# CristianSimion5/vk-raytracing-engine

Hardware: AMD Instinct MI355X
Metric: Mrays/s (higher is better)
Workload: dtype f32

## Files before the change

vk-raytracing-engine_amd/csrc/multihit.hip:

```cpp
#include <hip/hip_runtime.h>

#include "device_math.h"
#include "device_scene.h"
#include "kernels.h"
#include "query_common.h"
#include "traverse.h"
#include "traverse_wide.h"
#include "wf_streams.h"
#include "wide_node.h"

struct MultiList
{
  int* p;
  int K, cnt;
  float boundT;
  int boundGid;

  VKRT_DEV int& word(int f, int j) const { return p[(f * K + j) * 64]; }
  VKRT_DEV void begin(int* lanePtr, int k, float tmax)
  {
    p = lanePtr; K = k; cnt = 0; boundT = tmax; boundGid = -1;
  }
  VKRT_DEV bool admits(float t, int gid) const { return t < boundT || (t == boundT && gid < boundGid); }
  VKRT_DEV void insert(float t, int gid, int slot, float u, float v)
// ... 74 lines not shown
  tr.set(d);
  const float4* __restrict__ nodes = sc.nodes;
  const float4* __restrict__ tris = sc.tris;
  const int cap = (int)(sc.stackCap >> 1);
  const f3 id = mk3(safe_inv(d.x), safe_inv(d.y), safe_inv(d.z));
  const bool px = !(id.x < 0.0f), py = !(id.y < 0.0f), pz = !(id.z < 0.0f);
  const unsigned octinv = (px ? 1u : 0u) | (py ? 2u : 0u) | (pz ? 4u : 0u);
  uint2 G = make_uint2(0u, sc.rootRef == VKRT_TRAV_DONE ? 0u : 0x80000000u);
  int sp = 0;
  unsigned steps = sc.stepLimit;
  TravCount tc;
  while(G.y & 0xff000000u)
  {
    const unsigned bitIdx = 31u - (unsigned)__clz((int)G.y);
    const unsigned slot = (bitIdx - 24u) ^ octinv;
    const unsigned child = G.x + (unsigned)__popc(G.y & 0xffu & ((1u << slot) - 1u));
    G.y &= ~(1u << bitIdx);
    if(G.y & 0xff000000u)
    {
      if(sp < cap)
      {
        stk[sp * stride] = G;
        sp++;
      }
      else
        VKRT_TRAV_FAULT(sc);
    }
    if(--steps == 0u)
    {
      VKRT_TRAV_FAULT(sc);
      return;
    }
    uint2 T;
    w8_test_children<false, (TM & VKRT_TM_FILTER) != 0>(nodes, child, o, id, octinv * 0x01010101u, px, py, pz, tmin, L.boundT, G, T, tc,
                                                        query_node_masks<TM>(sc), query_cull_mask<TM>(sc));
    while(T.y != 0u)
    {
      const unsigned i = (unsigned)__ffs((int)T.y) - 1u;
      T.y &= T.y - 1u;
      if(--steps == 0u)
      {
        VKRT_TRAV_FAULT(sc);
        return;
      }
      multi_test_triangle<TM>(sc, tr, o, d, tmin, T.x + i, tris, L, raySeed);
    }
    if((G.y & 0xff000000u) == 0u)
    {
      if(sp == 0)
        return;
      sp--;
      G = stk[sp * stride];
    }
  }
}

template <bool WIDE, int TM>
__global__ __launch_bounds__(64)
void k_query_multi(const DevQueryScene sc, const float4* __restrict__ rays, uint64_t first, uint64_t n, uint32_t seed, int maxHits,
                   float4* __restrict__ hits, int* __restrict__ counts)
{
  extern __shared__ int lds_multi[];
  const uint64_t i = first + (uint64_t)blockIdx.x * 64u + threadIdx.x;
  if(i >= n)
    return;
  const float4 r0 = wfLoad(rays + 2 * i), r1 = wfLoad(rays + 2 * i + 1);
  const bool valid = queryRayValid(r0, r1) && (!(TM & VKRT_TM_FILTER) || sc.cullMask != 0u);
// ... 39 lines not shown
```

vk-raytracing-engine_amd/csrc/query.hip:

```cpp
#include <hip/hip_runtime.h>
#include <string.h>

#include "device_math.h"
#include "device_scene.h"
#include "kernels.h"
#include "query_common.h"
#include "traverse.h"
#include "traverse_wide.h"
#include "traverse_share.h"
#include "wf_streams.h"
#include "wide_node.h"

template <bool ANYHIT, bool WIDE, int TM>
__global__ __launch_bounds__(64)
__attribute__((amdgpu_waves_per_eu(TM != 0 && WIDE ? 5 : 1)))
void k_query(const DevQueryScene sc, const float4* __restrict__ rays, uint64_t first, uint64_t n, uint32_t seed, float4* __restrict__ hits,
             int* __restrict__ occ)
{
  extern __shared__ int lds_stack[];
  __shared__ int shareLds[VKRT_SHARE_LDS_WORDS];
  const uint64_t i = first + (uint64_t)blockIdx.x * 64u + threadIdx.x;
  const bool inRange = i < n;
  float4 r0 = make_float4(0.0f, 0.0f, 0.0f, 0.0f), r1 = make_float4(1.0f, 0.0f, 0.0f, 0.0f);
  if(inRange)
  {
    r0 = wfLoad(rays + 2 * i);
    r1 = wfLoad(rays + 2 * i + 1);
  }
  const bool valid = inRange && queryRayValid(r0, r1) && (!(TM & VKRT_TM_FILTER) || sc.cullMask != 0u);
  const unsigned long long validMask = __ballot(valid);
  RayHit hit;
  hit.t = r1.w; hit.u = 0.0f; hit.v = 0.0f; hit.slot = -1;
  TravCount tc;
  if(validMask != 0ull)
  {
    const f3 o = valid ? mk3(r0.x, r0.y, r0.z) : mk3(0.0f, 0.0f, 0.0f);
    const f3 d = valid ? mk3(r1.x, r1.y, r1.z) : mk3(1.0f, 0.0f, 0.0f);
    const float tmax = valid ? r1.w : 0.0f;
    const float tmin0 = __shfl(r0.w, __ffsll((long long)validMask) - 1);
    const bool share = WIDE && sc.shareMinIdle != 0u && sc.triThreshold != 0u && __ballot(valid && r0.w != tmin0) == 0ull;
    if(share)
    {
      uint2* stk = ((uint2*)lds_stack) + threadIdx.x;
      traverse_wide8_share<false, ANYHIT, TM>(sc, valid, o, d, tmin0, tmax, stk, shareRes(shareLds), hit, tc, seed);
    }
    else if(valid)
      traverse_any<false, WIDE, TM>(sc, o, d, r0.w, tmax, ANYHIT, lds_stack, (int)threadIdx.x, 64, hit, tc, seed);
  }
// ... 113 lines not shown
```

vk-raytracing-engine_amd/csrc/traverse_share.h:

```cpp
#pragma once
#include "traverse_wide.h"

#define VKRT_SHARE_LDS_WORDS 384
struct ShareRes
{
  unsigned long long* key;
  int* slot;
  float* u;
  float* v;
  int* donor;
};
VKRT_DEV void shareSync()
{
  __builtin_amdgcn_fence(__ATOMIC_RELEASE, "wavefront");
  __builtin_amdgcn_wave_barrier();
  __builtin_amdgcn_fence(__ATOMIC_ACQUIRE, "wavefront");
}
VKRT_DEV unsigned laneRank(unsigned long long mask)
{
  return __builtin_amdgcn_mbcnt_hi((unsigned)(mask >> 32), __builtin_amdgcn_mbcnt_lo((unsigned)mask, 0u));
}
VKRT_DEV ShareRes shareRes(int* lds320)
{
  ShareRes r;
  r.key = (unsigned long long*)lds320; r.slot = lds320 + 128; r.u = (float*)(lds320 + 192); r.v = (float*)(lds320 + 256); r.donor = lds320 + 320;
  return r;
}

template <bool COUNT, bool ANYHIT, int TM = 0>
VKRT_DEV void traverse_wide8_share(const DevScene& sc, bool valid, f3 o, f3 d, float tmin, float tmax, uint2* stk, ShareRes res, RayHit& hit,
                                   TravCount& tc, uint32_t raySeed = 0u)
{
  TriRay<(TM & VKRT_TM_WATERTIGHT) != 0> tr;
  tr.set(d);
  const float4* __restrict__ nodes = sc.nodes;
  const float4* __restrict__ tris = sc.tris;
  const int stride = 64;
  const int cap = (int)(sc.stackCap >> 1);
  const int lane = (int)lane_id();
  const unsigned shareMin = sc.shareMinIdle;
  bool farFirst = ANYHIT && anyhit_far_first(sc, o, d, tmax);

  res.key[lane] = ((unsigned long long)__float_as_uint(tmax) << 32) | 0xffffffffull;
  res.slot[lane] = -1; res.u[lane] = 0.0f; res.v[lane] = 0.0f;
  shareSync();

  int owner = lane;
  f3 id = mk3(safe_inv(d.x), safe_inv(d.y), safe_inv(d.z));
  bool px = !(id.x < 0.0f), py = !(id.y < 0.0f), pz = !(id.z < 0.0f);
  unsigned oct4 = ((px ? 1u : 0u) | (py ? 2u : 0u) | (pz ? 4u : 0u)) * 0x01010101u;
  uint2 G = make_uint2(0u, (valid && sc.rootRef != VKRT_TRAV_DONE) ? 0x80000000u : 0u);
  uint2 T = make_uint2(0u, 0u);
  int sp = 0, sb = 0, nPost = 0;
  unsigned steps = sc.stepLimit;
  bool busy = G.y != 0u;
  const bool lendOn = (TM & (VKRT_TM_WATERTIGHT | VKRT_TM_DISSOLVE)) != (VKRT_TM_WATERTIGHT | VKRT_TM_DISSOLVE) && (sc.shareFlags & VKRT_SHARE_TRI_LEND) != 0u;

  for(unsigned iter = 0;; iter++)
  {
    const unsigned long long busyMask = __ballot(busy);
    if(busyMask == 0ull)
      break;
    if((iter & sc.sharePeriodMask) == sc.sharePeriodMask && (unsigned)__popcll(~busyMask) >= shareMin)
    {
      const bool giveStack = busy && sp - sb >= 1;
      const bool giveChild = (sc.shareFlags & 1u) != 0u && busy && !giveStack && (G.y & 0xff000000u & ((G.y & 0xff000000u) - 1u)) != 0u;
      const bool mayTris = (sc.shareFlags & 16u) != 0u && busy && !giveStack && !giveChild;
      const bool giveParked = mayTris && nPost > 0;
      const bool giveTris = mayTris && !giveParked && (T.y & (T.y - 1u)) != 0u;
      const bool wants = giveStack || giveChild || giveParked || giveTris;
      const unsigned long long donorMask = __ballot(wants), idleMask = ~busyMask;
      if(donorMask != 0ull)
      {
        const unsigned n = min((unsigned)__popcll(donorMask), (unsigned)__popcll(idleMask));
        const unsigned giveRank = laneRank(donorMask), takeRank = laneRank(idleMask);
        const bool gives = wants && giveRank < n;
        const bool takes = !busy && takeRank < n;
        uint2 e = make_uint2(0u, 0u);
        if(gives)
        {
          if(giveStack)
          {
            e = stk[sb * stride];
            sb++;
          }
          else if(giveChild)
          {
            const unsigned top = G.y & 0xff000000u;
            const unsigned low = farFirst ? (0x80000000u >> (unsigned)__clz((int)top)) : (top & (0u - top));
            e = make_uint2(G.x, low | (G.y & 0xffu));
            G.y &= ~low;
          }
          else if(giveParked)
          {
            e = stk[(cap - nPost) * stride];
            e.x |= 0x80000000u;
            nPost--;
          }
          else
          {
            const unsigned lo = (unsigned)__ffs((int)T.y) - 1u, hi = 31u - (unsigned)__clz((int)T.y);
            const unsigned upper = T.y & ~((1u << ((lo + hi + 1u) >> 1)) - 1u);
            e = make_uint2(T.x | 0x80000000u, upper);
            T.y &= ~upper;
          }
          res.donor[giveRank] = lane;
        }
        shareSync();
        const int src = takes ? res.donor[takeRank] : lane;
        const unsigned ex = (unsigned)__shfl((int)e.x, src), ey = (unsigned)__shfl((int)e.y, src);
        const float ox = __shfl(o.x, src), oy = __shfl(o.y, src), oz = __shfl(o.z, src);
        const float dx = __shfl(d.x, src), dy = __shfl(d.y, src), dz = __shfl(d.z, src);
        const float ix = __shfl(id.x, src), iy = __shfl(id.y, src), iz = __shfl(id.z, src);
        const float tm = __shfl(tmax, src);
        const int ow = __shfl(owner, src);
        if(TM & VKRT_TM_DISSOLVE)
        {
          const uint32_t sd = (uint32_t)__shfl((int)raySeed, src);
          if(takes) raySeed = sd;
        }
        if(takes)
        {
          o = mk3(ox, oy, oz); d = mk3(dx, dy, dz); id = mk3(ix, iy, iz); tmax = tm;
          tr.set(d);
          farFirst = ANYHIT && anyhit_far_first(sc, o, d, tmax);
          px = !(id.x < 0.0f); py = !(id.y < 0.0f); pz = !(id.z < 0.0f);
          oct4 = ((px ? 1u : 0u) | (py ? 2u : 0u) | (pz ? 4u : 0u)) * 0x01010101u;
          if(ex & 0x80000000u)
          {
            G = make_uint2(0u, 0u);
            T = make_uint2(ex & 0x7fffffffu, ey);
          }
          else
          {
            G = make_uint2(ex, ey);
            T = make_uint2(0u, 0u);
          }
          sp = 0; sb = 0; nPost = 0;
          owner = ow;
          steps = sc.stepLimit;
          busy = true;
        }
      }
    }
    shareSync();
    if(busy || lendOn)
    {
      float bt = tmax;
      int bg = -1;
      bool finished = false;
      bool occluded = false;
      if(ANYHIT)
        finished = busy && __hip_atomic_load(&res.slot[owner], __ATOMIC_RELAXED, __HIP_MEMORY_SCOPE_WAVEFRONT) >= 0;
      else
      {
        const unsigned long long k = __hip_atomic_load(&res.key[owner], __ATOMIC_RELAXED, __HIP_MEMORY_SCOPE_WAVEFRONT);
        bt = __uint_as_float((unsigned)(k >> 32));
        bg = (int)(unsigned)k;
      }
      if(!finished)
      {
        struct Cand
        {
          bool found;
          float t, u, v;
          int slot, gid;
        };
        auto testOne = [&](Cand& cd) {
          const unsigned i = (unsigned)__ffs((int)T.y) - 1u;
          T.y &= T.y - 1u;
          const unsigned s = T.x + i;
          const float4* __restrict__ tp = tris + (size_t)s * VKRT_TRI_QUADS;
          const float4 a = tp[0];
          const float4 b = tp[1];
          const float4 c = tp[2];
          if(COUNT)
          {
            tc.tris++;
            if(lane == __ffsll((long long)__ballot(1)) - 1) tc.waveTriSteps++;
          }
          float t, u, v;
          bool ccw;
          if(tr.hit(o, d, a, b, c, t, u, v, ccw) && t > tmin)
          {
            if(ANYHIT)
            {
              if(t < tmax && !cd.found && !query_rejects<TM>(sc, c, ccw) && !anyhit_ignores<TM>(sc, s, c.y, raySeed, VKRT_HOOK_UV(TM, u, v)))
              {
                cd.found = true; cd.t = t; cd.slot = (int)s;
              }
            }
            else
            {
              const int gid = tri_gid<TM>(c.y);
              const float rt = cd.found ? cd.t : bt;
              const int rg = cd.found ? cd.gid : bg;
              if((t < rt || (t == rt && gid < rg)) && !query_rejects<TM>(sc, c, ccw) && !anyhit_ignores<TM>(sc, s, c.y, raySeed, VKRT_HOOK_UV(TM, u, v)))
              {
                cd.found = true; cd.t = t; cd.u = u; cd.v = v; cd.slot = (int)s; cd.gid = gid;
              }
            }
          }
        };
        auto publish = [&](const Cand& cd) {
          if(!cd.found)
            return;
          if(ANYHIT)
          {
            __hip_atomic_store(&res.slot[owner], cd.slot, __ATOMIC_RELAXED, __HIP_MEMORY_SCOPE_WAVEFRONT);
            occluded = true;
          }
          else
          {
            const unsigned long long mine = ((unsigned long long)__float_as_uint(cd.t) << 32) | (unsigned)cd.gid;
            __hip_atomic_fetch_min(&res.key[owner], mine, __ATOMIC_RELAXED, __HIP_MEMORY_SCOPE_WAVEFRONT);
            shareSync();
            if(__hip_atomic_load(&res.key[owner], __ATOMIC_RELAXED, __HIP_MEMORY_SCOPE_WAVEFRONT) == mine)
            {
              res.slot[owner] = cd.slot; res.u[owner] = cd.u; res.v[owner] = cd.v;
            }
            bt = cd.t; bg = cd.gid;
          }
        };
        auto flushT = [&]() {
          Cand cd = {false, 0.0f, 0.0f, 0.0f, -1, 0};
          while(T.y != 0u && !(ANYHIT && cd.found))
            testOne(cd);
          publish(cd);
        };
        if(G.y & 0xff000000u)
        {
          const unsigned bitIdx = farFirst ? (unsigned)__ffs((int)(G.y & 0xff000000u)) - 1u : 31u - (unsigned)__clz((int)G.y);
          const unsigned slot = (bitIdx - 24u) ^ (oct4 & 7u);
          const unsigned child = G.x + (unsigned)__popc(G.y & 0xffu & ((1u << slot) - 1u));
          G.y &= ~(1u << bitIdx);
          if(G.y & 0xff000000u)
          {
            if(__builtin_expect(sp + nPost >= cap && nPost > VKRT_W8_POSTPONE_ROOM, 0))
            {
              const uint2 keep = T;
              T = stk[(cap - nPost) * stride];
              nPost--;
              flushT();
              T = keep;
            }
            if(sp + nPost < cap)
            {
              stk[sp * stride] = G;
              sp++;
            }
            else
              VKRT_TRAV_FAULT(sc);
          }
          uint2 Tn;
          w8_test_children<COUNT, (TM & VKRT_TM_FILTER) != 0>(nodes, child, o, id, oct4, px, py, pz, tmin, bt, G, Tn, tc, query_node_masks<TM>(sc),
                                                              query_cull_mask<TM>(sc));
          if(Tn.y != 0u)
          {
            if(T.y != 0u)
            {
              if(__builtin_expect(nPost < VKRT_W8_MAX_POSTPONED && sp + nPost < cap, 1))
              {
                nPost++;
                stk[(cap - nPost) * stride] = T;
              }
              else
              {
                if(!occluded)
                  flushT();
                T.y = 0u;
              }
            }
            T = Tn;
          }
        }
        if((G.y & 0xff000000u) == 0u && sp > sb)
        {
          sp--;
          G = stk[sp * stride];
        }
        if(T.y == 0u && nPost > 0)
        {
          T = stk[(cap - nPost) * stride];
          nPost--;
        }
        bool triStep = true;
        if(sc.triThreshold > 1u)
          triStep = (unsigned)__popcll(__ballot(T.y != 0u)) * 64u >= sc.triThreshold * (unsigned)__popcll(busyMask) ||
                    __ballot((G.y & 0xff000000u) != 0u) == 0ull;
        bool lentStep = false;
        if(lendOn && triStep)
        {
          const bool tests = T.y != 0u && !occluded;
          const unsigned rest1 = T.y & (T.y - 1u);
          const bool multi = rest1 != 0u && !occluded, isFree = T.y == 0u && !occluded;
          const unsigned long long lendMask = __ballot(multi), freeMask = __ballot(isFree);
          const unsigned n = min((unsigned)__popcll(lendMask), (unsigned)__popcll(freeMask));
          if(n != 0u)
          {
            lentStep = true;
            const unsigned lendRank = laneRank(lendMask), freeRank = laneRank(freeMask);
            const bool borrows = isFree && freeRank < n;
            unsigned s = 0u, ls = 0u;
            if(multi && lendRank < n)
            {
              const unsigned hi = 31u - (unsigned)__clz((int)T.y);
              T.y &= ~(1u << hi);
              ls = T.x + hi;
              res.donor[lendRank] = lane;
            }
            if(tests)
            {
              s = T.x + (unsigned)__ffs((int)T.y) - 1u;
              T.y &= T.y - 1u;
            }
            shareSync();
            const int src = borrows ? res.donor[freeRank] : lane;
            const unsigned bs = (unsigned)__shfl((int)ls, src);
            const f3 ro = mk3(__shfl(o.x, src), __shfl(o.y, src), __shfl(o.z, src));
            const f3 rd = mk3(__shfl(d.x, src), __shfl(d.y, src), __shfl(d.z, src));
            const int row = __shfl(owner, src);
            const float rbt = __shfl(bt, src);
            const int rbg = ANYHIT ? 0 : __shfl(bg, src);
            uint32_t rseed = raySeed;
            if(TM & VKRT_TM_DISSOLVE)
              rseed = (uint32_t)__shfl((int)raySeed, src);
            if(tests || borrows)
            {
              if(borrows)
              {
                s = bs;
                tr.set(rd);
              }
              const float4* __restrict__ tp = tris + (size_t)s * VKRT_TRI_QUADS;
              const float4 a = tp[0];
              const float4 b = tp[1];
              const float4 c = tp[2];
              if(COUNT)
              {
                tc.tris++;
                if(lane == __ffsll((long long)__ballot(1)) - 1) tc.waveTriSteps++;
              }
              float t, u, v;
              bool ccw;
              if(tr.hit(ro, rd, a, b, c, t, u, v, ccw) && t > tmin)
              {
                if(ANYHIT)
                {
                  if(t < rbt && !query_rejects<TM>(sc, c, ccw) && !anyhit_ignores<TM>(sc, s, c.y, rseed, VKRT_HOOK_UV(TM, u, v)))
                  {
                    __hip_atomic_store(&res.slot[row], (int)s, __ATOMIC_RELAXED, __HIP_MEMORY_SCOPE_WAVEFRONT);
                    if(!borrows)
                      occluded = true;
                  }
                }
                else
                {
                  const int gid = tri_gid<TM>(c.y);
                  if((t < rbt || (t == rbt && gid < rbg)) && !query_rejects<TM>(sc, c, ccw) && !anyhit_ignores<TM>(sc, s, c.y, rseed, VKRT_HOOK_UV(TM, u, v)))
                  {
                    const unsigned long long mine = ((unsigned long long)__float_as_uint(t) << 32) | (unsigned)gid;
                    __hip_atomic_fetch_min(&res.key[row], mine, __ATOMIC_RELAXED, __HIP_MEMORY_SCOPE_WAVEFRONT);
                    shareSync();
                    if(__hip_atomic_load(&res.key[row], __ATOMIC_RELAXED, __HIP_MEMORY_SCOPE_WAVEFRONT) == mine)
                    {
                      res.slot[row] = (int)s; res.u[row] = u; res.v[row] = v;
                    }
                  }
                }
              }
              if((TM & VKRT_TM_WATERTIGHT) != 0 && borrows)
                tr.set(d);
            }
          }
        }
        if(!lentStep && T.y != 0u && triStep && !occluded)
        {
          Cand cd = {false, 0.0f, 0.0f, 0.0f, -1, 0};
          testOne(cd);
          publish(cd);
        }
        if(ANYHIT && occluded)
          finished = true;
        else if((G.y & 0xff000000u) == 0u && T.y == 0u && nPost == 0)
          finished = true;
        else if(--steps == 0u)
        {
          VKRT_TRAV_FAULT(sc);
          finished = true;
        }
      }
      if(finished)
      {
        if(lendOn && busy)
        {
          G.y = 0u; T.y = 0u; sp = 0; sb = 0; nPost = 0;
        }
        busy = false;
      }
    }
  }
  shareSync();
  hit.t = __uint_as_float((unsigned)(res.key[lane] >> 32)); hit.u = res.u[lane]; hit.v = res.v[lane]; hit.slot = res.slot[lane];
  if(ANYHIT)
    hit.t = tmax;
}
```

vk-raytracing-engine_amd/csrc/traverse_wide.h:

```cpp
#pragma once
#include "device_math.h"
#include "device_scene.h"
#include "traverse.h"
#include "wide_node.h"

typedef float vkrt_v4f __attribute__((ext_vector_type(4)));
VKRT_DEV float ubyte_f32(unsigned w, int k) { return (float)((w >> (8 * k)) & 0xffu); }

template <int TM>
struct W8State
{
  TriRay<(TM & VKRT_TM_WATERTIGHT) != 0> tr;
  uint32_t raySeed;
  bool farFirst;
  f3 o, d, id;
  float tmax, bestT, bestU, bestV;
  int bestSlot, bestGid;
  uint2 G;
  int sp;
  unsigned steps;
  bool anyHit;
};

template <int TM>
VKRT_DEV void w8_begin(const DevScene& sc, W8State<TM>& S, f3 o, f3 d, float tmax, bool anyHit, uint32_t raySeed)
{
  S.o = o; S.d = d;
  S.tr.set(d);
  S.raySeed = raySeed;
  S.farFirst = anyHit && anyhit_far_first(sc, o, d, tmax);
  S.id = mk3(safe_inv(d.x), safe_inv(d.y), safe_inv(d.z));
  S.tmax = tmax; S.bestT = tmax; S.bestU = 0.0f; S.bestV = 0.0f;
  S.bestSlot = -1; S.bestGid = -1;
  S.G = make_uint2(0u, sc.rootRef == VKRT_TRAV_DONE ? 0u : 0x80000000u);
  S.sp = 0;
  S.steps = sc.stepLimit;
  S.anyHit = anyHit;
}

VKRT_DEV unsigned w8_piece(unsigned idx4, unsigned bits4, int k)
{
#if defined(__HIP_DEVICE_COMPILE__) && !defined(__GFX9__)
  return ((bits4 >> (8 * k)) & 0xffu) << ((idx4 >> (8 * k)) & 31u);
#else
  unsigned r;
  if(k == 0)
    asm("v_lshlrev_b32_sdwa %0, %1, %2 dst_sel:DWORD dst_unused:UNUSED_PAD src0_sel:BYTE_0 src1_sel:BYTE_0" : "=v"(r) : "v"(idx4), "v"(bits4));
  else if(k == 1)
    asm("v_lshlrev_b32_sdwa %0, %1, %2 dst_sel:DWORD dst_unused:UNUSED_PAD src0_sel:BYTE_1 src1_sel:BYTE_1" : "=v"(r) : "v"(idx4), "v"(bits4));
  else if(k == 2)
    asm("v_lshlrev_b32_sdwa %0, %1, %2 dst_sel:DWORD dst_unused:UNUSED_PAD src0_sel:BYTE_2 src1_sel:BYTE_2" : "=v"(r) : "v"(idx4), "v"(bits4));
  else
    asm("v_lshlrev_b32_sdwa %0, %1, %2 dst_sel:DWORD dst_unused:UNUSED_PAD src0_sel:BYTE_3 src1_sel:BYTE_3" : "=v"(r) : "v"(idx4), "v"(bits4));
  return r;
#endif
}

template <bool COUNT, bool CULL = false>
VKRT_DEV void w8_test_children(const float4* __restrict__ nodes, unsigned child, f3 o, f3 id, unsigned oct4, bool px, bool py, bool pz, float tmin,
                               float bestT_in, uint2& G, uint2& T, TravCount& tc, const uint2* __restrict__ nodeMasks = nullptr,
                               unsigned cullMask = 0xffu)
{
  const float4* __restrict__ np = nodes + (size_t)child * VKRT_WNODE_QUADS;
  const float4 q0 = np[0], q1 = np[1], q2 = np[2], q3 = np[3], q4 = np[4];
  uint2 slotMasks = make_uint2(0xffffffffu, 0xffffffffu);
  if(CULL)
    slotMasks = nodeMasks[child];
  if(COUNT)
  {
    tc.nodes++;
    if((int)lane_id() == __ffsll((long long)__ballot(1)) - 1) tc.waveNodeSteps++;
  }
  const unsigned ew = __float_as_uint(q0.w);
  const unsigned imask = ew >> 24;
  const float asx = __uint_as_float((ew & 0xffu) << 23) * id.x;
  const float asy = __uint_as_float(((ew >> 8) & 0xffu) << 23) * id.y;
  const float asz = __uint_as_float(((ew >> 16) & 0xffu) << 23) * id.z;
  const float aox = (q0.x - o.x) * id.x, aoy = (q0.y - o.y) * id.y, aoz = (q0.z - o.z) * id.z;
  const float padx = VKRT_BOX_PAD_ABS * fmaf((float)VKRT_WNODE_QMAX, fabsf(asx), fabsf(aox));
  const float pady = VKRT_BOX_PAD_ABS * fmaf((float)VKRT_WNODE_QMAX, fabsf(asy), fabsf(aoy));
  const float padz = VKRT_BOX_PAD_ABS * fmaf((float)VKRT_WNODE_QMAX, fabsf(asz), fabsf(aoz));
  const float nox = aox - padx, fox = (aox + padx) * VKRT_BOX_PAD_REL2;
  const float noy = aoy - pady, foy = (aoy + pady) * VKRT_BOX_PAD_REL2;
  const float noz = aoz - padz, foz = (aoz + padz) * VKRT_BOX_PAD_REL2;
  const float fsx = asx * VKRT_BOX_PAD_REL2, fsy = asy * VKRT_BOX_PAD_REL2, fsz = asz * VKRT_BOX_PAD_REL2;
  const float nsx = asx, nsy = asy, nsz = asz;
  const unsigned lx0 = __float_as_uint(q2.x), lx1 = __float_as_uint(q2.y), ly0 = __float_as_uint(q2.z), ly1 = __float_as_uint(q2.w);
  const unsigned lz0 = __float_as_uint(q3.x), lz1 = __float_as_uint(q3.y), hx0 = __float_as_uint(q3.z), hx1 = __float_as_uint(q3.w);
  const unsigned hy0 = __float_as_uint(q4.x), hy1 = __float_as_uint(q4.y), hz0 = __float_as_uint(q4.z), hz1 = __float_as_uint(q4.w);
  const unsigned nx[2] = {px ? lx0 : hx0, px ? lx1 : hx1}, fx[2] = {px ? hx0 : lx0, px ? hx1 : lx1};
  const unsigned ny[2] = {py ? ly0 : hy0, py ? ly1 : hy1}, fy[2] = {py ? hy0 : ly0, py ? hy1 : ly1};
  const unsigned nz[2] = {pz ? lz0 : hz0, pz ? lz1 : hz1}, fz[2] = {pz ? hz0 : lz0, pz ? hz1 : lz1};
#define VKRT_WN_PLANE(a, w, k) ubyte_f32((a)[w], k)
  const float bestT = bestT_in;
  unsigned hitmask = 0u;
#pragma unroll
  for(int w = 0; w < 2; w++)
  {
    const unsigned meta4 = __float_as_uint(w == 0 ? q1.z : q1.w);
    const unsigned inner4 = (meta4 & (meta4 << 1)) & 0x10101010u;
    const unsigned innerMask4 = (inner4 >> 4) * 0x07u;
    const unsigned bitIndex4 = meta4 ^ (oct4 & innerMask4);
    const unsigned bits4 = (meta4 >> 5) & 0x07070707u;
#pragma unroll
    for(int k = 0; k < 4; k++)
    {
      const float tnx = fmaf(VKRT_WN_PLANE(nx, w, k), nsx, nox), tfx = fmaf(VKRT_WN_PLANE(fx, w, k), fsx, fox);
      const float tny = fmaf(VKRT_WN_PLANE(ny, w, k), nsy, noy), tfy = fmaf(VKRT_WN_PLANE(fy, w, k), fsy, foy);
      const float tnz = fmaf(VKRT_WN_PLANE(nz, w, k), nsz, noz), tfz = fmaf(VKRT_WN_PLANE(fz, w, k), fsz, foz);
      const float tn = fmaxf(fmaxf(tnx, tny), fmaxf(tnz, tmin));
      const float tf = fminf(fminf(tfx, tfy), fminf(tfz, bestT * VKRT_BOX_PAD_REL2));
      const unsigned piece = w8_piece(bitIndex4, bits4, k);
      if(CULL)
        hitmask |= (tn <= tf && (((w == 0 ? slotMasks.x : slotMasks.y) >> (8 * k)) & cullMask) != 0u) ? piece : 0u;
      else
        hitmask |= (tn <= tf) ? piece : 0u;
    }
  }
#undef VKRT_WN_PLANE
  G = make_uint2(__float_as_uint(q1.x), (hitmask & 0xff000000u) | imask);
  T = make_uint2(__float_as_uint(q1.y), hitmask & 0x00ffffffu);
}

template <bool COUNT, bool ANYHIT, int TM>
VKRT_DEV bool w8_iterate(const DevScene& sc, W8State<TM>& S, float tmin, uint2* stk, int stride, TravCount& tc)
{
  const float4* __restrict__ nodes = sc.nodes;
  const float4* __restrict__ tris = sc.tris;
  const int cap = (int)(sc.stackCap >> 1);
  const f3 o = S.o, d = S.d, id = S.id;
  const bool px = !(id.x < 0.0f), py = !(id.y < 0.0f), pz = !(id.z < 0.0f);
  const unsigned octinv = (px ? 1u : 0u) | (py ? 2u : 0u) | (pz ? 4u : 0u);
  uint2 G = S.G;
  uint2 T = make_uint2(0u, 0u);
  if(G.y & 0xff000000u)
  {
    const unsigned bitIdx = (ANYHIT && S.farFirst) ? (unsigned)__ffs((int)(G.y & 0xff000000u)) - 1u : 31u - (unsigned)__clz((int)G.y);
    const unsigned slot = (bitIdx - 24u) ^ octinv;
    const unsigned child = G.x + (unsigned)__popc(G.y & 0xffu & ((1u << slot) - 1u));
    G.y &= ~(1u << bitIdx);
    if(G.y & 0xff000000u)
    {
      if(S.sp < cap)
      {
        stk[S.sp * stride] = G;
        S.sp++;
      }
      else
        VKRT_TRAV_FAULT(sc);
    }
    if(--S.steps == 0u)
    {
      VKRT_TRAV_FAULT(sc);
      return false;
    }
    w8_test_children<COUNT, (TM & VKRT_TM_FILTER) != 0>(nodes, child, o, id, octinv * 0x01010101u, px, py, pz, tmin, S.bestT, G, T, tc,
                                                        query_node_masks<TM>(sc), query_cull_mask<TM>(sc));
  }
  while(T.y != 0u)
  {
    const unsigned i = (unsigned)__ffs((int)T.y) - 1u;
    T.y &= T.y - 1u;
    if(--S.steps == 0u)
    {
      VKRT_TRAV_FAULT(sc);
      return false;
    }
    const unsigned s = T.x + i;
    const float4* __restrict__ tp = tris + (size_t)s * VKRT_TRI_QUADS;
    const float4 a = tp[0];
    const float4 b = tp[1];
    const float4 c = tp[2];
    if(COUNT)
    {
      tc.tris++;
      if((int)lane_id() == __ffsll((long long)__ballot(1)) - 1) tc.waveTriSteps++;
    }
    float t, u, v;
    bool ccw;
    if(S.tr.hit(o, d, a, b, c, t, u, v, ccw))
    {
      if(t > tmin)
      {
        if(ANYHIT)
        {
          if(t < S.tmax && !query_rejects<TM>(sc, c, ccw) && !anyhit_ignores<TM>(sc, s, c.y, S.raySeed, VKRT_HOOK_UV(TM, u, v)))
          {
            S.bestSlot = (int)s;
            S.bestT = t;
            return false;
          }
        }
        else
        {
          const int gid = tri_gid<TM>(c.y);
          if((t < S.bestT || (t == S.bestT && gid < S.bestGid)) && !query_rejects<TM>(sc, c, ccw) && !anyhit_ignores<TM>(sc, s, c.y, S.raySeed, VKRT_HOOK_UV(TM, u, v)))
          {
            S.bestT = t; S.bestU = u; S.bestV = v; S.bestSlot = (int)s; S.bestGid = gid;
          }
        }
      }
    }
// ... 4 lines not shown
      return false;
    S.sp--;
    G = stk[S.sp * stride];
  }
  S.G = G;
  return true;
}

template <bool COUNT, bool ANYHIT, int TM>
VKRT_DEV void traverse_wide8_postpone(const DevScene& sc, f3 o, f3 d, float tmin, float tmax, uint2* stk, int stride, RayHit& hit, TravCount& tc,
                                      uint32_t raySeed)
{
  TriRay<(TM & VKRT_TM_WATERTIGHT) != 0> tr;
  tr.set(d);
  const bool farFirst = ANYHIT && anyhit_far_first(sc, o, d, tmax);
  const float4* __restrict__ nodes = sc.nodes;
  const float4* __restrict__ tris = sc.tris;
  const int cap = (int)(sc.stackCap >> 1);
  const unsigned thresh = sc.triThreshold;
  const f3 id = mk3(safe_inv(d.x), safe_inv(d.y), safe_inv(d.z));
  const bool px = !(id.x < 0.0f), py = !(id.y < 0.0f), pz = !(id.z < 0.0f);
  const unsigned octinv = (px ? 1u : 0u) | (py ? 2u : 0u) | (pz ? 4u : 0u);
  float bestT = tmax, bestU = 0.0f, bestV = 0.0f;
  int bestSlot = -1, bestGid = -1;
  uint2 G = make_uint2(0u, sc.rootRef == VKRT_TRAV_DONE ? 0u : 0x80000000u);
  uint2 T = make_uint2(0u, 0u);
  int sp = 0, nPost = 0;
  unsigned steps = sc.stepLimit;

  auto testOne = [&]() -> bool {
    const unsigned i = (unsigned)__ffs((int)T.y) - 1u;
    T.y &= T.y - 1u;
    const unsigned s = T.x + i;
    const float4* __restrict__ tp = tris + (size_t)s * VKRT_TRI_QUADS;
    const float4 a = tp[0];
    const float4 b = tp[1];
    const float4 c = tp[2];
    if(COUNT)
    {
      tc.tris++;
      if((int)lane_id() == __ffsll((long long)__ballot(1)) - 1) tc.waveTriSteps++;
    }
    float t, u, v;
    bool ccw;
    if(tr.hit(o, d, a, b, c, t, u, v, ccw) && t > tmin)
    {
      if(ANYHIT)
      {
        if(t < tmax && !query_rejects<TM>(sc, c, ccw) && !anyhit_ignores<TM>(sc, s, c.y, raySeed, VKRT_HOOK_UV(TM, u, v)))
        {
          bestSlot = (int)s; bestT = t;
          return true;
        }
      }
      else
      {
        const int gid = tri_gid<TM>(c.y);
        if((t < bestT || (t == bestT && gid < bestGid)) && !query_rejects<TM>(sc, c, ccw) && !anyhit_ignores<TM>(sc, s, c.y, raySeed, VKRT_HOOK_UV(TM, u, v)))
        {
          bestT = t; bestU = u; bestV = v; bestSlot = (int)s; bestGid = gid;
        }
      }
    }
    return false;
  };

  bool done = G.y == 0u;
// ... 1 lines not shown
  {
    if(G.y & 0xff000000u)
    {
      const unsigned bitIdx = farFirst ? (unsigned)__ffs((int)(G.y & 0xff000000u)) - 1u : 31u - (unsigned)__clz((int)G.y);
      const unsigned slot = (bitIdx - 24u) ^ octinv;
      const unsigned child = G.x + (unsigned)__popc(G.y & 0xffu & ((1u << slot) - 1u));
      G.y &= ~(1u << bitIdx);
      if(G.y & 0xff000000u)
      {
        if(__builtin_expect(sp + nPost >= cap && nPost > VKRT_W8_POSTPONE_ROOM, 0))
        {
          const uint2 keep = T;
          T = stk[(cap - nPost) * stride];
          nPost--;
          while(T.y != 0u)
            if(testOne())
            {
              done = true;
              break;
            }
          if(done)
            break;
          T = keep;
        }
        if(sp + nPost < cap)
        {
          stk[sp * stride] = G;
          sp++;
        }
        else
          VKRT_TRAV_FAULT(sc);
      }
      uint2 Tn;
      w8_test_children<COUNT, (TM & VKRT_TM_FILTER) != 0>(nodes, child, o, id, octinv * 0x01010101u, px, py, pz, tmin, bestT, G, Tn, tc,
                                                          query_node_masks<TM>(sc), query_cull_mask<TM>(sc));
      if(Tn.y != 0u)
      {
        if(T.y != 0u)
        {
          if(nPost < VKRT_W8_MAX_POSTPONED && sp + nPost < cap)
          {
            nPost++;
            stk[(cap - nPost) * stride] = T;
          }
          else
          {
            while(T.y != 0u)
              if(testOne())
              {
                done = true;
                break;
              }
            if(done)
              break;
          }
        }
        T = Tn;
      }
    }
    if((G.y & 0xff000000u) == 0u && sp > 0)
    {
      sp--;
      G = stk[sp * stride];
    }
    if(T.y == 0u && nPost > 0)
    {
      T = stk[(cap - nPost) * stride];
// ... 58 lines not shown
```

vk-raytracing-engine_amd/csrc/vkrt_api.cpp:

```cpp
#include <hip/hip_runtime.h>

#include <algorithm>
#include <chrono>
#include <cmath>
#include <cstdarg>
#include <cstdio>
#include <cstdlib>
#include <cstring>
#include <initializer_list>
#include <string>
#include <vector>

#include "../../include/vkrt.h"
#include "bvh_host.h"
#include "dev_buffer.h"
#include "device_scene.h"
#include "kernels.h"
#include "wide_node.h"

#define VKRT_TRI_THRESHOLD_DEFAULT 32
#define VKRT_WF_SHARE_DEFAULT 16
#define VKRT_WF_SHARE_FLAGS_DEFAULT 25
#define VKRT_WF_FRAMES_IN_FLIGHT_DEFAULT 3
#define VKRT_SPLIT_BUDGET_DEFAULT -1
// ... 1012 lines not shown
      return fail(rc, "%s build failed: %s", wantPloc ? "PLOC" : "LBVH", r.error.c_str());
    s->info.triangle_count = r.uniqueTris;
    s->dev.triCount = r.triCount;
    if(r.wide.buf.nodes.get())
      tree = std::move(r.wide);
    else if(wide && r.triCount > 0)
    {
      vkrt::BuiltBvh b2;
      b2.nodes.resize((size_t)r.tree.nodeCount * 16);
      std::vector<float> records((size_t)r.triCount * 12);
      hipError_t e = hipSuccess;
      if(r.tree.nodeCount) e = hipMemcpy(b2.nodes.data(), r.tree.buf.nodes.get(), b2.nodes.size() * 4, hipMemcpyDeviceToHost);
      if(e == hipSuccess) e = hipMemcpy(records.data(), r.tree.buf.tris.get(), records.size() * 4, hipMemcpyDeviceToHost);
      r.tree.buf = vkrt::TreeBuffers{};
      if(e != hipSuccess)
        return fail(VKRT_ERR_HIP, "LBVH download: %s", hipGetErrorString(e));
      b2.rootRef = r.tree.rootRef;
      b2.maxDepth = r.tree.maxDepth;
      b2.triOrder.resize(r.triCount);
      std::vector<vkrt::FlatTri> tris(r.triCount);
      for(uint32_t k = 0; k < r.triCount; k++)
      {
        b2.triOrder[k] = k;
        tris[k] = vkrt::unpack_triangle(&records[(size_t)k * 12], watertight);
      }
      vkrt::BuiltWide8 w8;
      vkrt::collapse_wide8(b2, tris, w8, watertight);
      if((rc = uploadHostTree(s, tris, nullptr, &w8, dissolvePtr, stream, tree)) != VKRT_OK)
        return rc;
    }
    else
      tree = std::move(r.tree);
  }
  installTree(s, tree);
  sceneBounds(s);
  if((rc = traversalSettings(s)) != VKRT_OK)
    return rc;
  if(s->dev.layout == 1u)
  {
    HIP_TRY(s->nodeMasks.alloc(std::max<size_t>(s->info.node_bytes / VKRT_WNODE_BYTES * 8, 16)));
    if((rc = computeNodeMasks(s, stream)) != VKRT_OK)
      return rc;
  }
  s->info.build_ms = std::chrono::duration<float, std::milli>(std::chrono::steady_clock::now() - t0).count();
  s->built = true;
  return VKRT_OK;
}

}

int vkrt_accel_build(vkrt_scene* s, uint32_t flags, void* hip_stream)
{
  if(!s)
    return fail(VKRT_ERR_INVALID_ARGUMENT, "scene is NULL");
  hipStream_t stream = (hipStream_t)hip_stream;
  if(s->positionsOnDevice)
  {
    int rc = setDevice(s);
    if(rc != VKRT_OK)
      return rc;
    HIP_TRY(hipDeviceSynchronize());
    if(!s->positions.empty())
      HIP_TRY(hipMemcpy(s->positions.data(), s->dev.positions, s->positions.size() * sizeof(float), hipMemcpyDeviceToHost));
    s->positionsOnDevice = false;
  }
  const bool deviceBuild = flags == 0 || (flags & (VKRT_BUILD_LBVH_GPU | VKRT_BUILD_PLOC_GPU)) != 0;
// ... 1083 lines not shown
```

vk-raytracing-engine_amd/csrc/wf_traverse.hip:

```cpp
#include <hip/hip_runtime.h>

#include "device_math.h"
#include "device_scene.h"
#include "kernels.h"
#include "rgen.h"
#include "traverse.h"
#include "traverse_wide.h"
#include "traverse_share.h"
#include "wf_streams.h"

enum { WF_K_CLOSEST_C = 0, WF_K_CLOSEST_P = 1, WF_K_SHADOW_S = 2, WF_K_SHADOW_P = 3 };

VKRT_DEV void storeHit(const TraceParams& P, const WfBuffers& B, int par, int kind, unsigned qi, const RayHit& hit)
{
  if(kind == WF_K_SHADOW_S)
    wfStore(rec(B, par, WF_S, WF_H0, qi), make_float4(0.0f, 0.0f, 0.0f, __int_as_float(hit.slot >= 0 ? 0 : -1)));
  else if(kind == WF_K_SHADOW_P)
    ((float*)rec(B, par, WF_P, WF_H0, qi))[0] = __int_as_float(hit.slot >= 0 ? 1 : 0);
  else
  {
    const int type = kind == WF_K_CLOSEST_C ? WF_C : WF_P;
    int inst = -1;
    if(hit.slot >= 0)
    {
      const uint4 ts = P.sc.triShade[hit.slot];
      inst = __float_as_int(P.sc.tris[hit.slot * VKRT_TRI_QUADS + 2].z);
      wfStore(rec(B, par, type, WF_H1, qi), make_float4(__uint_as_float(ts.x), __uint_as_float(ts.y), __uint_as_float(ts.z), __uint_as_float(ts.w)));
    }
    float* h = (float*)rec(B, par, type, WF_H0, qi);
    if(type == WF_C)
      wfStore(rec(B, par, WF_C, WF_H0, qi), make_float4(hit.t, hit.u, hit.v, __int_as_float(inst)));
    else
    {
      h[1] = hit.u; h[2] = hit.v; h[3] = __int_as_float(inst);
    }
  }
}

template <bool COUNT, bool WIDE, int TB, int TM = 0>
__global__ __launch_bounds__(TB)
__attribute__((amdgpu_waves_per_eu(TM != 0 && WIDE && TB == 64 ? 5 : 1)))
void k_wf_traverse(const TraceParams P, const WfBuffers B, const int round)
{
  extern __shared__ int lds_stack[];
  const int par = round & 1;
  const unsigned cC = *countOf(B, par, WF_C), cS = *countOf(B, par, WF_S), cP = *countOf(B, par, WF_P);
  if(blockIdx.x == 0 && threadIdx.x == 0)
  {
    for(int t = 0; t < WF_TYPES; t++) *countOf(B, par ^ 1, t) = 0u;
    if(cC + cP) atomicAdd(&P.counters->v[round % VKRT_COUNTER_SLOTS][0], (unsigned long long)cC + cP);
    if(cS + cP) atomicAdd(&P.counters->v[round % VKRT_COUNTER_SLOTS][1], (unsigned long long)cS + cP);
    if(cP) atomicAdd(&P.counters->v[round % VKRT_COUNTER_SLOTS][11], (unsigned long long)cP);
  }
  const unsigned nC = (cC + TB - 1) / TB, nP = (cP + TB - 1) / TB, nS = (cS + TB - 1) / TB;
  unsigned blk = blockIdx.x;
  int kind;
  unsigned count;
  if(blk < nC) { kind = WF_K_CLOSEST_C; count = cC; }
  else if((blk -= nC) < nP) { kind = WF_K_CLOSEST_P; count = cP; }
// ... 13 lines not shown
      r0.w = 10000.0f;
  }
  uint32_t raySeed = 0u;
  if((TM & VKRT_TM_DISSOLVE) && valid)
    raySeed = __float_as_uint(wfLoad(rec(B, par, type, WF_S0, qi)).w);
  TravCount tc;
  __shared__ int shareLds[VKRT_SHARE_LDS_WORDS];
  RayHit hit;
  if(WIDE && TB == 64 && P.sc.shareMinIdle != 0u && P.sc.triThreshold != 0u)
  {
    uint2* stk = ((uint2*)lds_stack) + threadIdx.x;
    if(anyHit)
      traverse_wide8_share<COUNT, true, TM>(P.sc, valid, mk3(r0.x, r0.y, r0.z), mk3(r1.x, r1.y, r1.z), 0.001f, r0.w, stk, shareRes(shareLds), hit, tc, raySeed);
    else
      traverse_wide8_share<COUNT, false, TM>(P.sc, valid, mk3(r0.x, r0.y, r0.z), mk3(r1.x, r1.y, r1.z), 0.001f, r0.w, stk, shareRes(shareLds), hit, tc, raySeed);
    if(valid)
      storeHit(P, B, par, kind, qi, hit);
  }
  else if(valid)
  {
    traverse_any<COUNT, WIDE, TM>(P.sc, mk3(r0.x, r0.y, r0.z), mk3(r1.x, r1.y, r1.z), 0.001f, r0.w, anyHit, lds_stack, (int)threadIdx.x, TB, hit, tc, raySeed);
    storeHit(P, B, par, kind, qi, hit);
  }
  if(COUNT)
  {
    __shared__ unsigned long long red[VKRT_COUNTER_STRIDE * (TB / 64)];
    const unsigned vals[10] = {0, 0, 0, 0, 0, 0, tc.nodes, tc.tris, tc.waveNodeSteps, tc.waveTriSteps};
    blockAddCounters(&P.counters->v[blockIdx.x % VKRT_COUNTER_SLOTS][0], vals, 10, red);
  }
}

template <bool COUNT, int TM>
__global__ __launch_bounds__(64)
__attribute__((amdgpu_waves_per_eu(TM != 0 ? 5 : 1)))
void k_wf_traverse_camera(const TraceParams P, const WfBuffers B, const int round, const int smpl)
{
  extern __shared__ int lds_stack[];
  const int par = round & 1;
  if(blockIdx.x == 0 && threadIdx.x == 0)
    for(int t = 0; t < WF_TYPES; t++) *countOf(B, par ^ 1, t) = 0u;
  const unsigned w = blockIdx.x * 64u + threadIdx.x;
  uint32_t x = 0, y = 0, lrow = 0;
  const bool valid = pixelOfWork(P, w, P.tileFirst, x, y, lrow);
  f3 o = mk3(0.0f), d = mk3(1.0f, 0.0f, 0.0f);
  uint32_t raySeed = 0u;
  if(valid)
  {
    LaneState L;
    bindPixel(P, L, x, lrow);
    L.prd.seed = smpl == 0 ? pixelSeed(P, x, y) : __float_as_uint(((const float*)(B.sampleState + pixelSlot(P, x, lrow)))[3]);
    L.smpl = smpl;
    startSample(P, L);
    o = L.prd.rayOrigin; d = L.prd.rayDirection;
    raySeed = L.prd.seed;
  }
  const unsigned nValid = (unsigned)__popcll(__ballot(valid));
  if(threadIdx.x == 0 && nValid)
  {
    atomicAdd(&P.counters->v[blockIdx.x % VKRT_COUNTER_SLOTS][0], (unsigned long long)nValid);
    if(smpl == 0) atomicAdd(&P.counters->v[blockIdx.x % VKRT_COUNTER_SLOTS][5], (unsigned long long)nValid);
  }
  TravCount tc;
  __shared__ int shareLds[VKRT_SHARE_LDS_WORDS];
  RayHit hit;
  uint2* stk = ((uint2*)lds_stack) + threadIdx.x;
  traverse_wide8_share<COUNT, false, TM>(P.sc, valid, o, d, 0.001f, 10000.0f, stk, shareRes(shareLds), hit, tc, raySeed);
  if(valid)
// ... 44 lines not shown
```

Measured before the change: 5454.

## Use 32-bit byte-offset addressing, LDS byte pointers, and raise waves-per-EU hints

Replaces 64-bit index arithmetic for node/triangle fetches with 32-bit byte offsets computed via v_lshl_add, and converts the shared traversal stack to LDS byte addresses with a global iteration bound instead of a per-lane step counter. It also computes the octant broadcast with a byte permute, simplifies the inner-child selection with a perm, and raises amdgpu_waves_per_eu to 6 for the default query and camera traversal kernels. The goal is to cut VGPR usage and ALU work so more waves fit per SIMD, at the cost of rejecting acceleration structures of 4 GiB or more and a slightly different step-limit fault semantic.

Result: no change. 5483, median of 4 (+0.5%).

```diff
diff --git a/vk-raytracing-engine_amd/csrc/multihit.hip b/vk-raytracing-engine_amd/csrc/multihit.hip
--- a/vk-raytracing-engine_amd/csrc/multihit.hip
+++ b/vk-raytracing-engine_amd/csrc/multihit.hip
@@ -130,7 +130,7 @@
       return;
     }
     uint2 T;
-    w8_test_children<false, (TM & VKRT_TM_FILTER) != 0>(nodes, child, o, id, octinv * 0x01010101u, px, py, pz, tmin, L.boundT, G, T, tc,
+    w8_test_children<false, (TM & VKRT_TM_FILTER) != 0>(nodes, child, o, id, w8_oct4(px, py, pz), px, py, pz, tmin, L.boundT, G, T, tc,
                                                         query_node_masks<TM>(sc), query_cull_mask<TM>(sc));
     while(T.y != 0u)
     {
diff --git a/vk-raytracing-engine_amd/csrc/query.hip b/vk-raytracing-engine_amd/csrc/query.hip
--- a/vk-raytracing-engine_amd/csrc/query.hip
+++ b/vk-raytracing-engine_amd/csrc/query.hip
@@ -12,8 +12,13 @@
 #include "wide_node.h"
 
 template <bool ANYHIT, bool WIDE, int TM>
+constexpr int queryWaves()
+{
+  return !WIDE ? 1 : (TM & (VKRT_TM_WATERTIGHT | VKRT_TM_DISSOLVE | VKRT_TM_ALPHA)) == 0 && !(ANYHIT && (TM & VKRT_TM_FILTER) != 0) ? 6 : TM != 0 ? 5 : 1;
+}
+template <bool ANYHIT, bool WIDE, int TM>
 __global__ __launch_bounds__(64)
-__attribute__((amdgpu_waves_per_eu(TM != 0 && WIDE ? 5 : 1)))
+__attribute__((amdgpu_waves_per_eu(queryWaves<ANYHIT, WIDE, TM>())))
 void k_query(const DevQueryScene sc, const float4* __restrict__ rays, uint64_t first, uint64_t n, uint32_t seed, float4* __restrict__ hits,
              int* __restrict__ occ)
 {
diff --git a/vk-raytracing-engine_amd/csrc/traverse_share.h b/vk-raytracing-engine_amd/csrc/traverse_share.h
--- a/vk-raytracing-engine_amd/csrc/traverse_share.h
+++ b/vk-raytracing-engine_amd/csrc/traverse_share.h
@@ -27,6 +27,22 @@
   return r;
 }
 
+#define VKRT_SHARE_ROW 512u
+typedef unsigned vkrt_v2u __attribute__((ext_vector_type(2)));
+typedef __attribute__((address_space(3))) vkrt_v2u ShareLdsEntry;
+VKRT_DEV unsigned shareColumn(uint2* stk) { return (unsigned)(size_t)(ShareLdsEntry*)stk; }
+VKRT_DEV uint2 shareLoad(unsigned at)
+{
+  const vkrt_v2u e = *(const ShareLdsEntry*)(size_t)at;
+  return make_uint2(e.x, e.y);
+}
+VKRT_DEV void shareStore(unsigned at, uint2 e)
+{
+  vkrt_v2u w;
+  w.x = e.x; w.y = e.y;
+  *(ShareLdsEntry*)(size_t)at = w;
+}
+
 template <bool COUNT, bool ANYHIT, int TM = 0>
 VKRT_DEV void traverse_wide8_share(const DevScene& sc, bool valid, f3 o, f3 d, float tmin, float tmax, uint2* stk, ShareRes res, RayHit& hit,
                                    TravCount& tc, uint32_t raySeed = 0u)
@@ -35,8 +51,9 @@
   tr.set(d);
   const float4* __restrict__ nodes = sc.nodes;
   const float4* __restrict__ tris = sc.tris;
-  const int stride = 64;
-  const int cap = (int)(sc.stackCap >> 1);
+  static_assert(VKRT_SHARE_ROW == 64u * sizeof(uint2), "one entry of every lane's column per row");
+  const unsigned capB = shareColumn(stk) + (sc.stackCap >> 1) * VKRT_SHARE_ROW;
+  const unsigned colBytes = (sc.stackCap >> 1) * VKRT_SHARE_ROW;
   const int lane = (int)lane_id();
   const unsigned shareMin = sc.shareMinIdle;
   bool farFirst = ANYHIT && anyhit_far_first(sc, o, d, tmax);
@@ -48,11 +65,11 @@
   int owner = lane;
   f3 id = mk3(safe_inv(d.x), safe_inv(d.y), safe_inv(d.z));
   bool px = !(id.x < 0.0f), py = !(id.y < 0.0f), pz = !(id.z < 0.0f);
-  unsigned oct4 = ((px ? 1u : 0u) | (py ? 2u : 0u) | (pz ? 4u : 0u)) * 0x01010101u;
+  unsigned oct4 = w8_oct4(px, py, pz);
   uint2 G = make_uint2(0u, (valid && sc.rootRef != VKRT_TRAV_DONE) ? 0x80000000u : 0u);
   uint2 T = make_uint2(0u, 0u);
-  int sp = 0, sb = 0, nPost = 0;
-  unsigned steps = sc.stepLimit;
+  unsigned sp = capB - colBytes, sb = sp, pt = capB;
+  const unsigned stepBound = min(sc.stepLimit, 0xffffffffu >> 6) << 6;
   bool busy = G.y != 0u;
   const bool lendOn = (TM & (VKRT_TM_WATERTIGHT | VKRT_TM_DISSOLVE)) != (VKRT_TM_WATERTIGHT | VKRT_TM_DISSOLVE) && (sc.shareFlags & VKRT_SHARE_TRI_LEND) != 0u;
 
@@ -61,12 +78,18 @@
     const unsigned long long busyMask = __ballot(busy);
     if(busyMask == 0ull)
       break;
+    if(__builtin_expect(iter == stepBound, 0))
+    {
+      if(busy)
+        VKRT_TRAV_FAULT(sc);
+      break;
+    }
     if((iter & sc.sharePeriodMask) == sc.sharePeriodMask && (unsigned)__popcll(~busyMask) >= shareMin)
     {
-      const bool giveStack = busy && sp - sb >= 1;
+      const bool giveStack = busy && sp != sb;
       const bool giveChild = (sc.shareFlags & 1u) != 0u && busy && !giveStack && (G.y & 0xff000000u & ((G.y & 0xff000000u) - 1u)) != 0u;
       const bool mayTris = (sc.shareFlags & 16u) != 0u && busy && !giveStack && !giveChild;
-      const bool giveParked = mayTris && nPost > 0;
+      const bool giveParked = mayTris && pt != capB;
       const bool giveTris = mayTris && !giveParked && (T.y & (T.y - 1u)) != 0u;
       const bool wants = giveStack || giveChild || giveParked || giveTris;
       const unsigned long long donorMask = __ballot(wants), idleMask = ~busyMask;
@@ -81,8 +104,8 @@
         {
           if(giveStack)
           {
-            e = stk[sb * stride];
-            sb++;
+            e = shareLoad(sb);
+            sb += VKRT_SHARE_ROW;
           }
           else if(giveChild)
           {
@@ -93,9 +116,9 @@
           }
           else if(giveParked)
           {
-            e = stk[(cap - nPost) * stride];
+            e = shareLoad(pt);
             e.x |= 0x80000000u;
-            nPost--;
+            pt += VKRT_SHARE_ROW;
           }
           else
           {
@@ -125,7 +148,7 @@
           tr.set(d);
           farFirst = ANYHIT && anyhit_far_first(sc, o, d, tmax);
           px = !(id.x < 0.0f); py = !(id.y < 0.0f); pz = !(id.z < 0.0f);
-          oct4 = ((px ? 1u : 0u) | (py ? 2u : 0u) | (pz ? 4u : 0u)) * 0x01010101u;
+          oct4 = w8_oct4(px, py, pz);
           if(ex & 0x80000000u)
           {
             G = make_uint2(0u, 0u);
@@ -136,9 +159,8 @@
             G = make_uint2(ex, ey);
             T = make_uint2(0u, 0u);
           }
-          sp = 0; sb = 0; nPost = 0;
+          sp = capB - colBytes; sb = sp; pt = capB;
           owner = ow;
-          steps = sc.stepLimit;
           busy = true;
         }
       }
@@ -170,7 +192,7 @@
           const unsigned i = (unsigned)__ffs((int)T.y) - 1u;
           T.y &= T.y - 1u;
           const unsigned s = T.x + i;
-          const float4* __restrict__ tp = tris + (size_t)s * VKRT_TRI_QUADS;
+          const float4* __restrict__ tp = treeAt(tris, treeTriBytes(s));
           const float4 a = tp[0];
           const float4 b = tp[1];
           const float4 c = tp[2];
@@ -236,18 +258,18 @@
           G.y &= ~(1u << bitIdx);
           if(G.y & 0xff000000u)
           {
-            if(__builtin_expect(sp + nPost >= cap && nPost > VKRT_W8_POSTPONE_ROOM, 0))
+            if(__builtin_expect(sp >= pt && pt + VKRT_W8_POSTPONE_ROOM * VKRT_SHARE_ROW < capB, 0))
             {
               const uint2 keep = T;
-              T = stk[(cap - nPost) * stride];
-              nPost--;
+              T = shareLoad(pt);
+              pt += VKRT_SHARE_ROW;
               flushT();
               T = keep;
             }
-            if(sp + nPost < cap)
-            {
-              stk[sp * stride] = G;
-              sp++;
+            if(sp < pt)
+            {
+              shareStore(sp, G);
+              sp += VKRT_SHARE_ROW;
             }
             else
               VKRT_TRAV_FAULT(sc);
@@ -259,10 +281,10 @@
           {
             if(T.y != 0u)
             {
-              if(__builtin_expect(nPost < VKRT_W8_MAX_POSTPONED && sp + nPost < cap, 1))
-              {
-                nPost++;
-                stk[(cap - nPost) * stride] = T;
+              if(__builtin_expect(capB - pt < VKRT_W8_MAX_POSTPONED * VKRT_SHARE_ROW && sp < pt, 1))
+              {
+                pt -= VKRT_SHARE_ROW;
+                shareStore(pt, T);
               }
               else
               {
@@ -274,15 +296,15 @@
             T = Tn;
           }
         }
-        if((G.y & 0xff000000u) == 0u && sp > sb)
-        {
-          sp--;
-          G = stk[sp * stride];
-        }
-        if(T.y == 0u && nPost > 0)
-        {
-          T = stk[(cap - nPost) * stride];
-          nPost--;
+        if((G.y & 0xff000000u) == 0u && sp != sb)
+        {
+          sp -= VKRT_SHARE_ROW;
+          G = shareLoad(sp);
+        }
+        if(T.y == 0u && pt != capB)
+        {
+          T = shareLoad(pt);
+          pt += VKRT_SHARE_ROW;
         }
         bool triStep = true;
         if(sc.triThreshold > 1u)
@@ -332,7 +354,7 @@
                 s = bs;
                 tr.set(rd);
               }
-              const float4* __restrict__ tp = tris + (size_t)s * VKRT_TRI_QUADS;
+              const float4* __restrict__ tp = treeAt(tris, treeTriBytes(s));
               const float4 a = tp[0];
               const float4 b = tp[1];
               const float4 c = tp[2];
@@ -382,19 +404,14 @@
         }
         if(ANYHIT && occluded)
           finished = true;
-        else if((G.y & 0xff000000u) == 0u && T.y == 0u && nPost == 0)
+        else if((G.y & 0xff000000u) == 0u && T.y == 0u && pt == capB)
           finished = true;
-        else if(--steps == 0u)
-        {
-          VKRT_TRAV_FAULT(sc);
-          finished = true;
-        }
       }
       if(finished)
       {
         if(lendOn && busy)
         {
-          G.y = 0u; T.y = 0u; sp = 0; sb = 0; nPost = 0;
+          G.y = 0u; T.y = 0u; sb = sp; pt = capB;
         }
         busy = false;
       }
diff --git a/vk-raytracing-engine_amd/csrc/traverse_wide.h b/vk-raytracing-engine_amd/csrc/traverse_wide.h
--- a/vk-raytracing-engine_amd/csrc/traverse_wide.h
+++ b/vk-raytracing-engine_amd/csrc/traverse_wide.h
@@ -6,6 +6,33 @@
 
 typedef float vkrt_v4f __attribute__((ext_vector_type(4)));
 VKRT_DEV float ubyte_f32(unsigned w, int k) { return (float)((w >> (8 * k)) & 0xffu); }
+
+static_assert(VKRT_WNODE_QUADS == 5 && VKRT_TRI_QUADS == 3, "treeNodeBytes / treeTriBytes scale by 80 and 48");
+VKRT_DEV unsigned treeNodeBytes(unsigned node)
+{
+#if defined(__HIP_DEVICE_COMPILE__)
+  unsigned r;
+  asm("v_lshl_add_u32 %0, %1, 2, %1" : "=v"(r) : "v"(node));
+  return r << 4;
+#else
+  return node * 80u;
+#endif
+}
+VKRT_DEV unsigned treeTriBytes(unsigned slot)
+{
+#if defined(__HIP_DEVICE_COMPILE__)
+  unsigned r;
+  asm("v_lshl_add_u32 %0, %1, 1, %1" : "=v"(r) : "v"(slot));
+  return r << 4;
+#else
+  return slot * 48u;
+#endif
+}
+template <class T>
+VKRT_DEV const T* treeAt(const T* __restrict__ base, unsigned byteOffset)
+{
+  return (const T*)((const char*)base + (size_t)byteOffset);
+}
 
 template <int TM>
 struct W8State
@@ -56,16 +83,22 @@
 #endif
 }
 
+VKRT_DEV unsigned w8_oct4(bool px, bool py, bool pz)
+{
+  const unsigned oct = (px ? 1u : 0u) | (py ? 2u : 0u) | (pz ? 4u : 0u);
+  return __builtin_amdgcn_perm(oct, oct, 0u);
+}
+
 template <bool COUNT, bool CULL = false>
 VKRT_DEV void w8_test_children(const float4* __restrict__ nodes, unsigned child, f3 o, f3 id, unsigned oct4, bool px, bool py, bool pz, float tmin,
                                float bestT_in, uint2& G, uint2& T, TravCount& tc, const uint2* __restrict__ nodeMasks = nullptr,
                                unsigned cullMask = 0xffu)
 {
-  const float4* __restrict__ np = nodes + (size_t)child * VKRT_WNODE_QUADS;
+  const float4* __restrict__ np = treeAt(nodes, treeNodeBytes(child));
   const float4 q0 = np[0], q1 = np[1], q2 = np[2], q3 = np[3], q4 = np[4];
   uint2 slotMasks = make_uint2(0xffffffffu, 0xffffffffu);
   if(CULL)
-    slotMasks = nodeMasks[child];
+    slotMasks = *treeAt(nodeMasks, child << 3);
   if(COUNT)
   {
     tc.nodes++;
@@ -98,9 +131,8 @@
   for(int w = 0; w < 2; w++)
   {
     const unsigned meta4 = __float_as_uint(w == 0 ? q1.z : q1.w);
-    const unsigned inner4 = (meta4 & (meta4 << 1)) & 0x10101010u;
-    const unsigned innerMask4 = (inner4 >> 4) * 0x07u;
-    const unsigned bitIndex4 = meta4 ^ (oct4 & innerMask4);
+    const unsigned leafSel4 = ~(meta4 & (meta4 >> 1)) & 0x08080808u;
+    const unsigned bitIndex4 = meta4 ^ __builtin_amdgcn_perm(oct4, oct4, leafSel4);
     const unsigned bits4 = (meta4 >> 5) & 0x07070707u;
 #pragma unroll
     for(int k = 0; k < 4; k++)
@@ -154,7 +186,7 @@
       VKRT_TRAV_FAULT(sc);
       return false;
     }
-    w8_test_children<COUNT, (TM & VKRT_TM_FILTER) != 0>(nodes, child, o, id, octinv * 0x01010101u, px, py, pz, tmin, S.bestT, G, T, tc,
+    w8_test_children<COUNT, (TM & VKRT_TM_FILTER) != 0>(nodes, child, o, id, w8_oct4(px, py, pz), px, py, pz, tmin, S.bestT, G, T, tc,
                                                         query_node_masks<TM>(sc), query_cull_mask<TM>(sc));
   }
   while(T.y != 0u)
@@ -167,7 +199,7 @@
       return false;
     }
     const unsigned s = T.x + i;
-    const float4* __restrict__ tp = tris + (size_t)s * VKRT_TRI_QUADS;
+    const float4* __restrict__ tp = treeAt(tris, treeTriBytes(s));
     const float4 a = tp[0];
     const float4 b = tp[1];
     const float4 c = tp[2];
@@ -238,7 +270,7 @@
     const unsigned i = (unsigned)__ffs((int)T.y) - 1u;
     T.y &= T.y - 1u;
     const unsigned s = T.x + i;
-    const float4* __restrict__ tp = tris + (size_t)s * VKRT_TRI_QUADS;
+    const float4* __restrict__ tp = treeAt(tris, treeTriBytes(s));
     const float4 a = tp[0];
     const float4 b = tp[1];
     const float4 c = tp[2];
@@ -306,7 +338,7 @@
           VKRT_TRAV_FAULT(sc);
       }
       uint2 Tn;
-      w8_test_children<COUNT, (TM & VKRT_TM_FILTER) != 0>(nodes, child, o, id, octinv * 0x01010101u, px, py, pz, tmin, bestT, G, Tn, tc,
+      w8_test_children<COUNT, (TM & VKRT_TM_FILTER) != 0>(nodes, child, o, id, w8_oct4(px, py, pz), px, py, pz, tmin, bestT, G, Tn, tc,
                                                           query_node_masks<TM>(sc), query_cull_mask<TM>(sc));
       if(Tn.y != 0u)
       {
diff --git a/vk-raytracing-engine_amd/csrc/vkrt_api.cpp b/vk-raytracing-engine_amd/csrc/vkrt_api.cpp
--- a/vk-raytracing-engine_amd/csrc/vkrt_api.cpp
+++ b/vk-raytracing-engine_amd/csrc/vkrt_api.cpp
@@ -1068,6 +1068,9 @@
     else
       tree = std::move(r.tree);
   }
+  if(tree.nodeBytes >= (1ull << 32) || tree.triangleBytes >= (1ull << 32))
+    return fail(VKRT_ERR_UNSUPPORTED, "the acceleration structure reaches 4 GiB (nodes %llu bytes, triangles %llu bytes): the traversal addresses each "
+                "array with 32-bit byte offsets", (unsigned long long)tree.nodeBytes, (unsigned long long)tree.triangleBytes);
   installTree(s, tree);
   sceneBounds(s);
   if((rc = traversalSettings(s)) != VKRT_OK)
diff --git a/vk-raytracing-engine_amd/csrc/wf_traverse.hip b/vk-raytracing-engine_amd/csrc/wf_traverse.hip
--- a/vk-raytracing-engine_amd/csrc/wf_traverse.hip
+++ b/vk-raytracing-engine_amd/csrc/wf_traverse.hip
@@ -23,8 +23,8 @@
     int inst = -1;
     if(hit.slot >= 0)
     {
-      const uint4 ts = P.sc.triShade[hit.slot];
-      inst = __float_as_int(P.sc.tris[hit.slot * VKRT_TRI_QUADS + 2].z);
+      const uint4 ts = *treeAt(P.sc.triShade, (unsigned)hit.slot << 4);
+      inst = __float_as_int(treeAt(P.sc.tris, treeTriBytes((unsigned)hit.slot))[2].z);
       wfStore(rec(B, par, type, WF_H1, qi), make_float4(__uint_as_float(ts.x), __uint_as_float(ts.y), __uint_as_float(ts.z), __uint_as_float(ts.w)));
     }
     float* h = (float*)rec(B, par, type, WF_H0, qi);
@@ -104,7 +104,7 @@
 
 template <bool COUNT, int TM>
 __global__ __launch_bounds__(64)
-__attribute__((amdgpu_waves_per_eu(TM != 0 ? 5 : 1)))
+__attribute__((amdgpu_waves_per_eu(COUNT ? (TM != 0 ? 5 : 1) : 6)))
 void k_wf_traverse_camera(const TraceParams P, const WfBuffers B, const int round, const int smpl)
 {
   extern __shared__ int lds_stack[];
```
